# JorisAR/GDPathTracing

Measured on AMD Instinct MI355X. Metric: Mrays/sec at 1920x1080, 8 spp, 4 bounces, higher is better.
Workload: dtype f32

## Files before the change

gdpathtracing_amd/csrc/jpt_kernels_wf2.hip:

```cpp
#include <algorithm>
#include <cstdlib>

#include "jpt_trace_core.h"
#include "jpt_tie_walk.h"
#include "jpt_tuning.h"

#ifndef JPT_PRIMARY_WAVES
#define JPT_PRIMARY_WAVES 7
#endif

namespace jpt {

namespace {

constexpr int kBlock = kTraceBlock;
constexpr uint32_t kSegments = 256u * JPT_WAVES_PER_SIMD;
struct WfTune {
    int refill_idle;
    int primary_refill_idle;
    int node_min_lanes;
    int leaf_min_lanes;
    int inst_min_lanes;
    int phase_frac16;
    int tail_rounds;
    int tail_lanes;
};

template <bool COUNT, bool W4>
__device__ __forceinline__ bool walk_round(Traversal<COUNT, W4>& tr, bool active, const WideSceneDev& sc,
                                           const typename Traversal<COUNT, W4>::Stack& st, DevCounters& cnt, const WfTune& tune, uint32_t& steps)
{
    const int kNodeMinLanes = tune.node_min_lanes;
    const bool lane0 = (threadIdx.x & 63) == 0;
    if (COUNT && lane0) cnt.phase[0]++;
    const int na = __popcll(__ballot(active));
    const int cap = (na * tune.phase_frac16) >> 4;
    const int lmin = tune.leaf_min_lanes < cap ? tune.leaf_min_lanes : cap;
    const int imin = tune.inst_min_lanes < cap ? tune.inst_min_lanes : cap;
    for (int it = 0; it < 64; it++) {
        if (active && !tr.have && tr.sp > 0) tr.pop_next(st);
        const bool want = active && tr.wants_node();
        const unsigned long long m = __ballot(want);
        if (m == 0 || (it > 0 && __popcll(m) < kNodeMinLanes)) break;
        if (COUNT && lane0) {
            cnt.phase[1]++;
            cnt.phase[2] += (unsigned long long)__popcll(m);
        }
        if (want) tr.node_step(sc, st, cnt);
        if (COUNT && want) steps++;
    }
    bool wl = active && tr.wants_leaf();
    bool wi = active && tr.wants_instance();
    if (W4 && (tune.leaf_min_lanes > 1 || tune.inst_min_lanes > 1)) {
        const int nl = __popcll(__ballot(wl)), ni = __popcll(__ballot(wi));
        const bool nodes_left = __any(active && tr.wants_node()) || __any(active && !tr.have && tr.sp > 0);
        const bool run_l = nl >= lmin || !(nodes_left || ni >= imin);
        const bool run_i = ni >= imin || !(nodes_left || (run_l && nl > 0));
        wl = wl && run_l;
        wi = wi && run_i;
    }
    if (COUNT) {
        const int nl = __popcll(__ballot(wl)), ni = __popcll(__ballot(wi));
        if (lane0 && nl) {
            cnt.phase[3]++;
            cnt.phase[4] += (unsigned long long)nl;
        }
        if (lane0 && ni) {
            cnt.phase[5]++;
            cnt.phase[6] += (unsigned long long)ni;
        }
    }
    if (wl) tr.leaf_step(sc, cnt);
    if (wi) tr.instance_step(sc, st, cnt);
    if (COUNT && (wl || wi)) steps++;
    return active && tr.finished();
}

__device__ __forceinline__ bool in_mask(const unsigned long long m) { return __builtin_amdgcn_inverse_ballot_w64(m); }

template <bool COUNT, bool W4>
__device__ __forceinline__ unsigned long long walk_round_masked(Traversal<COUNT, W4>& tr, const unsigned long long act, const WideSceneDev& sc,
                                                                const typename Traversal<COUNT, W4>::Stack& st, DevCounters& cnt, const WfTune& tune,
                                                                uint32_t& steps)
{
    const int kNodeMinLanes = tune.node_min_lanes;
    const bool lane0 = (threadIdx.x & 63) == 0;
    const bool active = in_mask(act);
    if (COUNT && lane0) cnt.phase[0]++;
    const int na = __popcll(act);
    const int cap = (na * tune.phase_frac16) >> 4;
    const int lmin = tune.leaf_min_lanes < cap ? tune.leaf_min_lanes : cap;
    const int imin = tune.inst_min_lanes < cap ? tune.inst_min_lanes : cap;
    for (int it = 0; it < 64; it++) {
        if (active && !tr.have && tr.sp > 0) tr.template pop_next<true>(st);
        const bool want = active && tr.wants_node();
        const unsigned long long m = __ballot(want);
        if (m == 0 || (it > 0 && __popcll(m) < kNodeMinLanes)) break;
        if (COUNT && lane0) {
            cnt.phase[1]++;
            cnt.phase[2] += (unsigned long long)__popcll(m);
        }
        if (want) tr.node_step(sc, st, cnt);
        if (COUNT && want) steps++;
    }
    const unsigned long long hm = __ballot(tr.have), bm = __ballot(tr.in_blas);
    const unsigned long long lf = __ballot(tr.cur < 0), sm = __ballot(tr.sp > 0);
    const unsigned long long hv = act & hm;
    unsigned long long wlm = hv & lf & bm, wim = hv & lf & ~bm;
    if (W4 && (tune.leaf_min_lanes > 1 || tune.inst_min_lanes > 1)) {
        const int nl = __popcll(wlm), ni = __popcll(wim);
        const bool nodes_left = ((hv & ~lf) | (act & ~hm & sm)) != 0ull;
        const bool run_l = nl >= lmin || !(nodes_left || ni >= imin);
        const bool run_i = ni >= imin || !(nodes_left || (run_l && nl > 0));
        wlm = run_l ? wlm : 0ull;
        wim = run_i ? wim : 0ull;
    }
    if (COUNT) {
        const int nl = __popcll(wlm), ni = __popcll(wim);
        if (lane0 && nl) {
            cnt.phase[3]++;
            cnt.phase[4] += (unsigned long long)nl;
        }
        if (lane0 && ni) {
            cnt.phase[5]++;
            cnt.phase[6] += (unsigned long long)ni;
        }
    }
    const bool wl = in_mask(wlm), wi = in_mask(wim);
    if (wl) tr.leaf_step(sc, cnt);
    if (wi) tr.instance_step(sc, st, cnt);
    if (COUNT && (wl || wi)) steps++;
    return act & ~((hm & ~wlm) | wim) & ~sm;
}

typedef float jpt_v4f __attribute__((ext_vector_type(4)));
typedef uint32_t jpt_v4u __attribute__((ext_vector_type(4)));
__device__ __forceinline__ float4 stream_ld4(const float4* p)
{
    const jpt_v4f v = __builtin_nontemporal_load(reinterpret_cast<const jpt_v4f*>(p));
    return make_float4(v.x, v.y, v.z, v.w);
}
__device__ __forceinline__ void stream_st4(float4* p, const float4 v)
{
    jpt_v4f w;
    w.x = v.x; w.y = v.y; w.z = v.z; w.w = v.w;
    __builtin_nontemporal_store(w, reinterpret_cast<jpt_v4f*>(p));
}
__device__ __forceinline__ uint4 stream_ldu4(const uint4* p)
{
    const jpt_v4u v = __builtin_nontemporal_load(reinterpret_cast<const jpt_v4u*>(p));
    return make_uint4(v.x, v.y, v.z, v.w);
}
__device__ __forceinline__ void stream_stf(float* p, const float v) { __builtin_nontemporal_store(v, p); }
__device__ __forceinline__ uint32_t stream_ldu(const uint32_t* p) { return __builtin_nontemporal_load(p); }
__device__ __forceinline__ void stream_stu(uint32_t* p, const uint32_t v) { __builtin_nontemporal_store(v, p); }

constexpr uint32_t kHasRadiance = 0x80000000u;
constexpr uint32_t kPathMask = 0x7fffffffu;

struct Wf2Buffers {
    float4* ray_o[2];
    float4* ray_d[2];
    float4* hit_a;
    uint32_t* hit_b;
    float4* thr_q[2];
    float4* thr;
    float4* rad;
    uint32_t* fin8;
    float* first_depth;
    uint32_t* qcount;
    uint32_t* redo_count;
    float4* redo_rec;
    uint32_t redo_cap;
};

struct FastDiv {
    uint32_t d, m;
};
inline FastDiv make_fastdiv(uint32_t d) { return FastDiv{d ? d : 1u, d > 1u ? (uint32_t)(0x100000000ull / d) : 0xffffffffu}; }
__device__ __forceinline__ uint32_t fdiv(uint32_t n, const FastDiv& f)
{
    uint32_t q = __umulhi(n, f.m);
    const uint32_t r = n - q * f.d;
    return r >= f.d ? q + 1u : q;
}

struct Wf2Dims {
    int32_t tile_x0, tile_y0;
    int32_t tiles_x, tiles_y;
    int32_t full_tiles_x, full_tiles_y;
    uint32_t tiles_per_frame;
    uint32_t slots_per_frame;
    uint32_t n_chunks;
    uint32_t seg_cap;
    uint32_t run_shift;
    FastDiv by_tiles_x, by_full_tiles_x;
    FastDiv by_frames;
    int32_t acc_groups = 1;
};

__device__ __forceinline__ void slot_to_pixel(uint32_t slot, const Wf2Dims& dm, int& px, int& ly)
{
    const uint32_t tile = slot >> 6, lane = slot & 63u;
    const uint32_t ty = fdiv(tile, dm.by_tiles_x), tx = tile - ty * (uint32_t)dm.tiles_x;
    const uint32_t ix = lane & 7u, iy = lane >> 3;
    px = (int)((tx + (uint32_t)dm.tile_x0) * 8u + ix);
    ly = (int)((ty + (uint32_t)dm.tile_y0) * 8u + iy);
}

__device__ __forceinline__ void path_slot_frame(uint32_t path, const Wf2Dims& dm, uint32_t n_frames, uint32_t& slot, uint32_t& f)
{
    slot = fdiv(path, dm.by_frames);
    f = path - slot * n_frames;
}

// ... 99 lines not shown
                const uint32_t lim = want < room ? want : room;
                if (give && r < lim) {
                    tr.sp--;
                    pw(2u * (n_pool + r)) = top;
                    pw(2u * (n_pool + r) + 1u) = (int32_t)((tr.in_blas ? 1u : 0u) | (tr.cur_inst << 1));
                }
                const uint32_t given = (uint32_t)__popcll(gm);
                n_pool += given < lim ? given : lim;
            }
        }
        __builtin_amdgcn_fence(__ATOMIC_RELEASE, "wavefront");
        __builtin_amdgcn_wave_barrier();
    }
    if (COUNT) {
        for (int off = 32; off > 0; off >>= 1) my_steps += (uint32_t)__shfl_xor((int)my_steps, off);
        if (lane == 0) count_walk(cnt, my_steps);
    }
    const float best = wave_min_f(tr.hit.t);
    const unsigned long long win = __ballot(tr.hit.tri != kNone && tr.hit.t == best);
    TraceHit out;
    out.t = 1e9f;
    out.u = out.v = 0.0f;
    out.tri = out.inst = 0u;
    out.front = false;
    if (win && best < 1e9f) {
        unsigned long long pick = win;
        if (__popcll(win) > 1) {
            const bool mine = ((win >> lane) & 1ull) != 0ull;
            uint32_t kt = mine ? tr.hit.tri : 0u;
            for (int off = 32; off > 0; off >>= 1) {
                const uint32_t o = (uint32_t)__shfl_xor((int)kt, off);
                kt = o > kt ? o : kt;
            }
            const bool top = mine && tr.hit.tri == kt;
            uint32_t ki = top ? ((tr.hit.inst >> kInstBits) & kInstMask) : 0u;
            for (int off = 32; off > 0; off >>= 1) {
                const uint32_t o = (uint32_t)__shfl_xor((int)ki, off);
                ki = o > ki ? o : ki;
            }
            pick = __ballot(top && ((tr.hit.inst >> kInstBits) & kInstMask) == ki);
        }
        const int w = __ffsll((long long)pick) - 1;
        out.t = best;
        out.u = __shfl(tr.hit.u, w);
        out.v = __shfl(tr.hit.v, w);
        out.tri = (uint32_t)__shfl((int)tr.hit.tri, w);
        out.front = __shfl((int)tr.hit.front, w) != 0;
        const uint32_t wi = (uint32_t)__shfl((int)tr.hit.inst, w);
        const uint32_t found_in = (wi >> kInstBits) & kInstMask;
        const bool tied = __popcll(win) > 1 || (wi & kHitTied) != 0u;
        out.inst = found_in | (found_in << kInstBits) | (tied ? kHitTied : 0u);
    }
    return out;
}

template <bool COUNT>
__device__ __attribute__((noinline)) void coop_walk_call(const WideSceneDev* __restrict__ scp, int32_t* lds_col, int32_t* pool, float ox, float oy,
                                                         float oz, float dx, float dy, float dz, DevCounters* cntp, TraceHit* out)
{
    int32_t spill[kStackSpill + 2];
    const typename Traversal<COUNT, true>::Stack st{lds_col, spill, kTraceBlock, kStackLds - 2, kStackSpill + 2};
    const WideSceneDev sc = *scp;
    DevCounters none = {};
    *out = coop_walk<COUNT>(sc, st, pool, mk3(ox, oy, oz), mk3(dx, dy, dz), COUNT ? *cntp : none, (uint32_t)kTraceBlock);
}


#ifndef JPT_MAX_CHAIN
#define JPT_MAX_CHAIN 4
#endif
constexpr int kMaxChain = JPT_MAX_CHAIN;
template <bool COUNT, bool W4, bool TAIL>
__device__ __forceinline__ void trace_queue(const WideSceneDev& sc, const Wf2Buffers& wb, const Wf2Dims& dm, const int bounce, const WfTune& tune,
                                            const uint32_t seg0, const uint32_t (&end)[kMaxChain], const uint32_t n, int32_t* __restrict__ stack,
                                            uint32_t* __restrict__ s_cursor, DevCounters& cnt)
{
    const int lane = threadIdx.x & 63;
    int32_t spill[kStackSpill];
    const typename Traversal<COUNT, W4>::Stack my_stack{&stack[threadIdx.x], spill, kTraceBlock, kStackLds};
    uint32_t dry_rounds = 0;
    const float4* __restrict__ qo = wb.ray_o[bounce & 1];
    const float4* __restrict__ qd = wb.ray_d[bounce & 1];
    Traversal<COUNT, W4> tr;
    tr.have = tr.in_blas = false;
    tr.cur = 0;
    tr.sp = 0;
    unsigned long long act = 0ull, unsaved = 0ull;
    bool exhausted = false;
    size_t my_loc = 0;
    uint32_t walk_steps = 0;
    auto save_hit = [&]() {
        stream_st4(&wb.hit_a[my_loc], make_float4(tr.hit.t, tr.hit.u, tr.hit.v, __uint_as_float(tr.hit.tri)));
        stream_stu(&wb.hit_b[my_loc], tr.hit.inst | (tr.hit.front ? 0x80000000u : 0u));
    };

    for (;;) {
        const unsigned long long idle = ~act;
        const int n_idle = __popcll(idle);
        if (!exhausted && n_idle >= tune.refill_idle) {
            if (in_mask(unsaved)) save_hit();
            unsaved = 0ull;
            uint32_t start = 0;
            if (lane == 0) start = atomicAdd(s_cursor, (uint32_t)n_idle);
            start = (uint32_t)__builtin_amdgcn_readfirstlane((int)start);
            if (start + (uint32_t)n_idle >= n) exhausted = true;
            if (start < n) {
                const uint32_t idx = start + lanes_below(idle, lane);
                const unsigned long long fill = idle & __ballot(idx < n);
                if (in_mask(fill)) {
                    uint32_t k = 0, first = 0;
                    for (int j = 0; j < kMaxChain - 1; j++)
                        if (idx >= end[j]) {
                            k = (uint32_t)j + 1u;
                            first = end[j];
                        }
                    const size_t loc = (size_t)(seg0 + k) * dm.seg_cap + (idx - first);
                    const float4 ro = stream_ld4(&qo[loc]), rd = stream_ld4(&qd[loc]);
                    tr.begin(sc, mk3(ro.x, ro.y, ro.z), mk3(rd.x, rd.y, rd.z));
                    my_loc = loc;
                    walk_steps = 0;
                }
                act |= fill;
            }
        }
        if (act == 0ull) {
            if (exhausted) break;
            continue;
        }
        {
            const unsigned long long done = walk_round_masked<COUNT, W4>(tr, act, sc, my_stack, cnt, tune, walk_steps);
            act &= ~done;
            unsaved |= done;
            if (COUNT) {
                if (in_mask(done)) count_walk(cnt, walk_steps);
            }
            if constexpr (TAIL && W4) {
                if (exhausted && ++dry_rounds >= (uint32_t)tune.tail_rounds && __popcll(act) <= tune.tail_lanes) break;
            }
        }
    }
    if constexpr (TAIL && W4) {
        unsigned long long left = act;
        if (left) {
            if (in_mask(unsaved)) save_hit();
            unsaved = 0ull;
            const int wave_col = (int)(threadIdx.x & ~63u);
            while (left) {
                const int src = __ffsll((long long)left) - 1;
                left &= left - 1ull;
                TraceHit h;
                const WideSceneDev sc_tail = sc;
                coop_walk_call<COUNT>(&sc_tail, &stack[threadIdx.x], &stack[(kStackLds - 2) * kTraceBlock + wave_col], __shfl(tr.wo.x, src),
                                      __shfl(tr.wo.y, src), __shfl(tr.wo.z, src), __shfl(tr.wd.x, src), __shfl(tr.wd.y, src), __shfl(tr.wd.z, src),
                                      COUNT ? &cnt : nullptr, &h);
                if (lane == src) {
                    tr.hit = h;
                    save_hit();
                }
            }
        }
    }
    if (in_mask(unsaved)) save_hit();
}

template <bool COUNT, bool W4, bool TAIL = false>
__global__ __launch_bounds__(kBlock, JPT_WAVES_PER_SIMD) void wf2_trace(WideSceneDev sc, Wf2Buffers wb, Wf2Dims dm, int bounce, WfTune tune,
                                                    int chain, DevCounters* __restrict__ counters)
{
    __shared__ int32_t stack[kStackLds * kBlock];
    __shared__ uint32_t s_cursor;
    const uint32_t seg0 = blockIdx.x * (uint32_t)chain;
    uint32_t end[kMaxChain];
    uint32_t n = 0;
    for (int k = 0; k < kMaxChain; k++) {
        if (k < chain && seg0 + (uint32_t)k < kSegments) n += wb.qcount[(size_t)bounce * kSegments + seg0 + (uint32_t)k];
        end[k] = n;
    }
    if (n == 0) return;
    if (threadIdx.x == 0) s_cursor = 0;
    __syncthreads();
    DevCounters cnt = {};
    trace_queue<COUNT, W4, TAIL>(sc, wb, dm, bounce, tune, seg0, end, n, stack, &s_cursor, cnt);
    if (COUNT) flush_counters(cnt, counters);
}

constexpr float kCellMargin = 0.01f;
__device__ __forceinline__ bool sky_cells_at(const RefCamera& cam, float two_over_w, float two_over_h, float fx, float fy, float w_ref, float& w_out,
                                             float v[3], f3& d)
{
    d = raster_direction_approx(cam, two_over_w, two_over_h, fx, fy, w_out);
    const f3 c = mk3(0.0f, 0.0f, 0.0f) + mk3(1.0f, 1.0f, 1.0f) * sample_sky(d);
    v[0] = clamp_(c.x, 0.0f, 1.0f) * 255.0f + 0.5f;
    v[1] = clamp_(c.y, 0.0f, 1.0f) * 255.0f + 0.5f;
    v[2] = clamp_(c.z, 0.0f, 1.0f) * 255.0f + 0.5f;
    return (w_out * w_ref > 0.0f) && (d.y == d.y);
}
__device__ __forceinline__ float sky_interior_excess(const f3 c[4])
{
    float chord2 = 0.0f, ay = 0.0f;
    for (int i = 0; i < 4; i++) {
        ay = fmax_(ay, __builtin_fabsf(c[i].y));
        for (int j = i + 1; j < 4; j++) {
            const f3 e = c[i] - c[j];
            chord2 = fmax_(chord2, e.x * e.x + e.y * e.y + e.z * e.z);
        }
    }
    if (!(chord2 < 0.2f)) return 1e30f;
    const float theta2 = 1.1f * chord2;
    const float m = fmin_(1.0f, ay + __builtin_sqrtf(theta2));
    return 6.4f * 0.25f * theta2 * m;
}

__global__ __launch_bounds__(kBlock) void wf2_sky_tiles(Wf2Dims dm, FrameParams fp, RefCamera cam, uint32_t* __restrict__ tile_cell)
// ... 523 lines not shown
```

gdpathtracing_amd/csrc/jpt_trace_core.h:

```cpp
#pragma once

#include "jpt_kernels.h"
#include "jpt_shade.h"

namespace jpt {

constexpr int kTraceBlock = 256;
#ifndef JPT_STACK_LDS
#define JPT_STACK_LDS 20
#endif
#ifndef JPT_WAVES_PER_SIMD
#define JPT_WAVES_PER_SIMD 7
#endif
constexpr int kStackLds = JPT_STACK_LDS;
constexpr int kStackSpill = 76;
constexpr int32_t kSentinel = 0x7fffffff;

struct WideSceneDev {
    const WideNode* __restrict__ blas_nodes;
    const WideNode* __restrict__ tlas_nodes;
    const WideNodeQ* __restrict__ nodesq;
    const WideTri* __restrict__ tris;
    const WideInstance* __restrict__ instances;
    int32_t tlas_root;
    uint32_t n_instances;
    const ReachTri* __restrict__ reach_tri;
    const ReachInst* __restrict__ reach_inst;
};

__device__ __forceinline__ float4 ld4(const void* p) { return *reinterpret_cast<const float4*>(p); }

__device__ __forceinline__ float slab(const f3& o, const f3& rD, float mnx, float mny, float mnz, float mxx, float mxy, float mxz)
{
    const float tx1 = (mnx - o.x) * rD.x, tx2 = (mxx - o.x) * rD.x;
    float tmin = fmin_(tx1, tx2), tmax = fmax_(tx1, tx2);
    const float ty1 = (mny - o.y) * rD.y, ty2 = (mxy - o.y) * rD.y;
    tmin = fmax_(tmin, fmin_(ty1, ty2)), tmax = fmin_(tmax, fmax_(ty1, ty2));
    const float tz1 = (mnz - o.z) * rD.z, tz2 = (mxz - o.z) * rD.z;
    tmin = fmax_(tmin, fmin_(tz1, tz2)), tmax = fmin_(tmax, fmax_(tz1, tz2));
    return (tmax >= tmin && tmax > 0.0f) ? tmin : 1e30f;
}

constexpr int kInstBits = 15;
constexpr uint32_t kInstMask = (1u << kInstBits) - 1u;
constexpr uint32_t kHitTied = 1u << 30;

struct TraceHit {
    float t, u, v;
    uint32_t tri, inst;
    bool front;
};

template <bool COUNT, bool W4 = false, bool REACH = false>
struct Traversal {
    static constexpr bool kLean = W4;
    f3 wo, wd, wrD;
    f3 o, d, rD;
    f3 ood;
    f3 xrD;
    TraceHit hit;
    int32_t cur;
    int sp;
    uint32_t cur_inst;
    bool in_blas, have;

    struct Stack {
        int32_t* __restrict__ lds;
        int32_t* __restrict__ spill;
        int stride = kTraceBlock;
        int lds_entries = kStackLds;
        int spill_entries = kStackSpill;
    };

    __device__ __forceinline__ void push(const Stack& st, int32_t v)
    {
        if (sp < st.lds_entries) st.lds[sp * st.stride] = v;
        else if (sp < st.lds_entries + st.spill_entries) st.spill[sp - st.lds_entries] = v;
        sp++;
    }
    __device__ __forceinline__ int32_t pop(const Stack& st)
    {
        sp--;
        if (st.lds_entries <= 0) return sp < st.spill_entries ? st.spill[sp] : kSentinel;
        const int row = sp < st.lds_entries ? sp : st.lds_entries - 1;
        int32_t v = st.lds[row * st.stride];
        if (__builtin_expect(sp >= st.lds_entries, 0)) v = sp < st.lds_entries + st.spill_entries ? st.spill[sp - st.lds_entries] : kSentinel;
        return v;
    }

    __device__ __forceinline__ void begin(const WideSceneDev& sc, f3 ro, f3 rd)
    {
        wo = ro;
        wd = rd;
        o = ro;
        d = rd;
        set_level();
        wrD = (kLean && REACH) ? xrD : rD;
        hit.t = 1e9f;
        hit.u = hit.v = 0.0f;
        hit.tri = hit.inst = 0;
        hit.front = false;
        sp = 0;
        in_blas = false;
        cur_inst = 0;
        cur = sc.tlas_root;
        have = sc.n_instances != 0;
    }

    __device__ __forceinline__ void set_level()
    {
        if (kLean) {
            rD = mk3(__builtin_amdgcn_fmed3f(__builtin_amdgcn_rcpf(d.x), -kRcpClamp, kRcpClamp), __builtin_amdgcn_fmed3f(__builtin_amdgcn_rcpf(d.y), -kRcpClamp, kRcpClamp),
                     __builtin_amdgcn_fmed3f(__builtin_amdgcn_rcpf(d.z), -kRcpClamp, kRcpClamp));
            ood = mk3(-(o.x * rD.x), -(o.y * rD.y), -(o.z * rD.z));
            if (REACH) xrD = rcp3(d);
        } else {
            rD = rcp3(d);
        }
    }


    __device__ __forceinline__ bool wants_node() const { return have && cur >= 0; }
    __device__ __forceinline__ bool wants_leaf() const { return have && cur < 0 && in_blas; }
    __device__ __forceinline__ bool wants_instance() const { return have && cur < 0 && !in_blas; }
    __device__ __forceinline__ bool finished() const { return !have && sp == 0; }

    __device__ __forceinline__ void node_step4(const WideSceneDev& sc, const Stack& st, DevCounters& cnt)
    {
        const char* __restrict__ base = reinterpret_cast<const char*>(sc.nodesq);
        const uint32_t rec = (uint32_t)cur << 6;
        const float4 h0 = ld4(base + rec);
        const float4 h1 = ld4(base + (rec + 16u));
        const float4 h2 = ld4(base + (rec + 32u));
        const float4 cf = ld4(base + (rec + 48u));
        node_step4_rec(h0, h1, h2, cf, st, cnt);
    }
    __device__ __forceinline__ void node_step4_rec(const float4 h0, const float4 h1, const float4 h2, const float4 cf, const Stack& st, DevCounters& cnt)
    {
        if (COUNT) {
            if (in_blas) cnt.blas_expand++;
            else cnt.tlas_expand++;
        }
        const float ax = h0.w * rD.x, ay = h1.x * rD.y, az = h1.y * rD.z;
        const float bx = __builtin_fmaf(h0.x, rD.x, ood.x), by = __builtin_fmaf(h0.y, rD.y, ood.y), bz = __builtin_fmaf(h0.z, rD.z, ood.z);
        const float mx = __builtin_fmaf(kWalkSlackOverEps, __builtin_fabsf(ax), __builtin_fabsf(bx)) + __builtin_fabsf(ood.x);
        const float my = __builtin_fmaf(kWalkSlackOverEps, __builtin_fabsf(ay), __builtin_fabsf(by)) + __builtin_fabsf(ood.y);
        const float mz = __builtin_fmaf(kWalkSlackOverEps, __builtin_fabsf(az), __builtin_fabsf(bz)) + __builtin_fabsf(ood.z);
        const float nbx = __builtin_fmaf(-kWalkEps, mx, bx), fbx = __builtin_fmaf(kWalkEps, mx, bx);
        const float nby = __builtin_fmaf(-kWalkEps, my, by), fby = __builtin_fmaf(kWalkEps, my, by);
        const float nbz = __builtin_fmaf(-kWalkEps, mz, bz), fbz = __builtin_fmaf(kWalkEps, mz, bz);
        const bool negx = __float_as_int(d.x) < 0, negy = __float_as_int(d.y) < 0, negz = __float_as_int(d.z) < 0;
        const uint32_t lox = __float_as_uint(h1.z), loy = __float_as_uint(h1.w), loz = __float_as_uint(h2.x);
        const uint32_t hix = __float_as_uint(h2.y), hiy = __float_as_uint(h2.z), hiz = __float_as_uint(h2.w);
        const uint32_t nwx = negx ? hix : lox, fwx = negx ? lox : hix;
        const uint32_t nwy = negy ? hiy : loy, fwy = negy ? loy : hiy;
        const uint32_t nwz = negz ? hiz : loz, fwz = negz ? loz : hiz;
        int32_t r0 = __float_as_int(cf.x), r1 = __float_as_int(cf.y), r2 = __float_as_int(cf.z), r3 = __float_as_int(cf.w);
        constexpr uint32_t kInvalid = 0x7f800000u;
        const float tcur = hit.t;
        auto key = [&](int k, int32_t ch) -> uint32_t {
            const float qnx = (float)((nwx >> (8 * k)) & 255u), qny = (float)((nwy >> (8 * k)) & 255u), qnz = (float)((nwz >> (8 * k)) & 255u);
            const float qfx = (float)((fwx >> (8 * k)) & 255u), qfy = (float)((fwy >> (8 * k)) & 255u), qfz = (float)((fwz >> (8 * k)) & 255u);
            const float t_in = fmax_(fmax_(fmax_(__builtin_fmaf(qnx, ax, nbx), __builtin_fmaf(qny, ay, nby)), __builtin_fmaf(qnz, az, nbz)), 0.0f);
            const float t_out = fmin_(fmin_(fmin_(__builtin_fmaf(qfx, ax, fbx), __builtin_fmaf(qfy, ay, fby)), __builtin_fmaf(qfz, az, fbz)), tcur);
            return ((t_in <= t_out) & (ch != kEmptyChild)) ? __float_as_uint(t_in) : kInvalid;
        };
        uint32_t k0 = key(0, r0), k1 = key(1, r1), k2 = key(2, r2), k3 = key(3, r3);
        auto cswap = [](uint32_t& ka, uint32_t& kb, int32_t& ra, int32_t& rb) {
            const bool lt = ka < kb;
            const uint32_t klo = lt ? ka : kb, khi = lt ? kb : ka;
            const int32_t rlo = lt ? ra : rb, rhi = lt ? rb : ra;
            ka = klo; kb = khi; ra = rlo; rb = rhi;
        };
        cswap(k0, k1, r0, r1);
        cswap(k2, k3, r2, r3);
        cswap(k0, k2, r0, r2);
        cswap(k1, k3, r1, r3);
        cswap(k1, k2, r1, r2);
        have = k0 < kInvalid;
        cur = have ? r0 : cur;
        if (k1 < kInvalid) {
            if (k2 < kInvalid) {
                if (k3 < kInvalid) push(st, r3);
                push(st, r2);
            }
            push(st, r1);
        }
    }

    __device__ __forceinline__ void node_step(const WideSceneDev& sc, const Stack& st, DevCounters& cnt)
    {
        if (W4) {
            node_step4(sc, st, cnt);
            return;
        }
        const WideNode* n = (in_blas ? sc.blas_nodes : sc.tlas_nodes) + cur;
        const float4 a = ld4(&n->lmin[0]);
        const float4 b = ld4(&n->lmax[1]);
        const float4 c = ld4(&n->rmin[2]);
        const float4 e = ld4(&n->left);
        if (COUNT) {
            if (in_blas) cnt.blas_expand++;
            else cnt.tlas_expand++;
        }
        const float d1 = slab(o, rD, a.x, a.y, a.z, a.w, b.x, b.y);
        const float d2 = slab(o, rD, b.z, b.w, c.x, c.y, c.z, c.w);
        const int32_t left = __float_as_int(e.x), right = __float_as_int(e.y);
        const bool lv = d1 < hit.t, rv = d2 < hit.t;
        const bool left_first = d1 < d2;
        const int32_t near_ref = left_first ? left : right, far_ref = left_first ? right : left;
        const bool near_v = left_first ? lv : rv, far_v = left_first ? rv : lv;
        have = false;
        if (near_v) {
            if (far_v) push(st, far_ref);
            cur = near_ref;
            have = true;
        } else if (far_v) {
            cur = far_ref;
            have = true;
        }
    }

    __device__ __forceinline__ void leaf_step(const WideSceneDev& sc, DevCounters& cnt)
    {
        const uint32_t bits = (uint32_t)~cur;
        const uint32_t first = bits & kLeafFirstMask;
        const uint32_t count = (bits >> kLeafCountShift) + 1u;
        have = false;
        for (uint32_t i = 0; i < count; i++) {
            const uint32_t ti = first + i;
            const WideTri* tp = sc.tris + ti;
            const float4 q0 = ld4(&tp->v0[0]);
            const float4 q1 = ld4(&tp->e1[0]);
            const float4 q2 = ld4(&tp->e2[0]);
            if (COUNT) cnt.tri_tests++;
            const f3 v0 = mk3(q0.x, q0.y, q0.z), edge1 = mk3(q1.x, q1.y, q1.z), edge2 = mk3(q2.x, q2.y, q2.z);
            if (W4) {
                const f3 pvec = cross3(d, edge2);
                const float det = dot3(edge1, pvec);
                const float invDet = 1.0f / det;
                const f3 tvec = o - v0;
                const float u = dot3(tvec, pvec) * invDet;
                const f3 qvec = cross3(tvec, edge1);
                const float v = dot3(d, qvec) * invDet;
                const float t = dot3(edge2, qvec) * invDet;
                bool out = (__builtin_fabsf(det) < 1e-5f) | (u < 0.0f) | (u > 1.0f) | (v < 0.0f) | (u + v > 1.0f) |
                           (t < 0.0f) | (t > hit.t);
                if (REACH) {
                    if (!out && !reaches_triangle(sc, ti)) out = true;
                }
                float facing = dot3(mk3(q0.w, q1.w, q2.w), d);
                asm volatile("" : "+v"(facing));
                const bool front = facing > 0.0f;
                if (!out) {
                    const bool closer = t < hit.t;
                    hit.inst = ((closer ? cur_inst : hit.inst) & kInstMask) | (cur_inst << kInstBits) | (closer ? 0u : kHitTied);
                    hit.t = t;
                    hit.u = u;
                    hit.v = v;
                    hit.tri = ti;
                    hit.front = front;
                }
            } else {
                const f3 pvec = cross3(d, edge2);
                const float det = dot3(edge1, pvec);
                if (__builtin_fabsf(det) < 1e-5f) continue;
                const float invDet = 1.0f / det;
                const f3 tvec = o - v0;
                const float u = dot3(tvec, pvec) * invDet;
                if (u < 0.0f || u > 1.0f) continue;
                const f3 qvec = cross3(tvec, edge1);
                const float v = dot3(d, qvec) * invDet;
                if (v < 0.0f || u + v > 1.0f) continue;
                const float t = dot3(edge2, qvec) * invDet;
                if (t < 0.0f || t > hit.t) continue;
                if (REACH) {
                    if (!reaches_triangle(sc, ti)) continue;
                }
                hit.inst = (((t < hit.t) ? cur_inst : hit.inst) & kInstMask) | (cur_inst << kInstBits);
                hit.t = t;
                hit.u = u;
                hit.v = v;
                hit.tri = ti;
                hit.front = dot3(cross3(edge1, edge2), d) > 0.0f;
            }
        }
    }

    __device__ __forceinline__ bool reaches_triangle(const WideSceneDev& sc, uint32_t ti) const
    {
        const float4 a = ld4(&sc.reach_tri[ti].lo[0]), b = ld4(&sc.reach_tri[ti].hi[0]);
        if (__float_as_uint(a.w) != 0u) return true;
        return slab(o, kLean ? xrD : rD, a.x, a.y, a.z, b.x, b.y, b.z) < 1e30f;
    }

    __device__ __forceinline__ void instance_step(const WideSceneDev& sc, const Stack& st, DevCounters& cnt)
    {
        cur_inst = (uint32_t)~cur;
        if (REACH) {
            if (sc.n_instances > 1u) {
                const float4 a = ld4(&sc.reach_inst[cur_inst].lo[0]), b = ld4(&sc.reach_inst[cur_inst].hi[0]);
                if (!(slab(wo, wrD, a.x, a.y, a.z, b.x, b.y, b.z) < 1e30f)) {
                    if (kLean) {
                        o = wo;
                        d = wd;
                        set_level();
                    }
                    have = false;
                    return;
                }
            }
        }
        const WideInstance* ip = sc.instances + cur_inst;
        const float4 m0 = ld4(&ip->inv[0]);
        const float4 m1 = ld4(&ip->inv[4]);
        const float4 m2 = ld4(&ip->inv[8]);
        const int32_t root = ip->root;
        if (COUNT) cnt.inst_visits++;
        o = mk3(m0.x * wo.x + m0.w * wo.y + m1.z * wo.z + m2.y, m0.y * wo.x + m1.x * wo.y + m1.w * wo.z + m2.z,
                m0.z * wo.x + m1.y * wo.y + m2.x * wo.z + m2.w);
        d = mk3(m0.x * wd.x + m0.w * wd.y + m1.z * wd.z, m0.y * wd.x + m1.x * wd.y + m1.w * wd.z,
                m0.z * wd.x + m1.y * wd.y + m2.x * wd.z);
        set_level();
        in_blas = true;
        push(st, kSentinel);
        cur = root;
        have = true;
    }

    template <bool ON_DEMAND = false>
    __device__ __forceinline__ void pop_next(const Stack& st)
    {
        cur = pop(st);
        if (cur == kSentinel) {
            in_blas = false;
            if (sp == 0) return;
            cur = pop(st);
            if (!kLean || cur >= 0) {
                o = wo;
                d = wd;
                if (kLean && ON_DEMAND) asm volatile("" : "+v"(d.x), "+v"(d.y), "+v"(d.z));
                if (kLean) set_level();
                else rD = wrD;
            }
        }
        have = true;
    }

    __device__ __forceinline__ bool step(const WideSceneDev& sc, const Stack& st, DevCounters& cnt)
    {
        if (!have) {
            if (sp == 0) return false;
            pop_next(st);
            if (!have) return false;
        }
        if (cur >= 0) node_step(sc, st, cnt);
        else if (in_blas) leaf_step(sc, cnt);
        else instance_step(sc, st, cnt);
        return true;
    }
};

}
```

gdpathtracing_amd/csrc/jpt_wf2_paths.h:

```cpp
#if JPT_ENV >= 3
#if JPT_ENV == 4
#define JPT_ENV_NAME(name) name##_tx
#define JPT_LTOTAL (lt.n != 0u ? lt.marg[lt.n_blocks] : 0.0f)
#define JPT_MISS_WEIGHT env_miss_weight_tx
#define JPT_HIT_WEIGHT light_hit_weight_tx
#else
#define JPT_ENV_NAME(name) name##_lt
#define JPT_LTOTAL lt.marg[lt.n_blocks]
#define JPT_MISS_WEIGHT env_miss_weight
#define JPT_HIT_WEIGHT light_hit_weight
#endif
#define JPT_ENV_PARAM , EnvDev env, EnvSampDev es, LightDev lt, Wf2Nee nee, Wf2Nee lnee, int env_mode
#define JPT_ENV_ARG , env, es, lt, nee, lnee, env_mode
#define JPT_NEE_PARAM , bool& shadow, float4& so, float4& sd, float4& sc4, bool& lshadow, float4& lso, float4& lsd, float4& lsc
#define JPT_NEE_ARG , shadow, so, sd, sc4, lshadow, lso, lsd, lsc
#define JPT_SKY(d) (env_mode != 0 ? env_radiance(env, d) : sample_sky(d))
#define JPT_PDF lnee.pdf
#elif JPT_ENV == 2
#define JPT_ENV_NAME(name) name##_mis
#define JPT_ENV_PARAM , EnvDev env, EnvSampDev es, Wf2Nee nee
#define JPT_ENV_ARG , env, es, nee
#define JPT_NEE_PARAM , bool& shadow, float4& so, float4& sd, float4& sc4
#define JPT_NEE_ARG , shadow, so, sd, sc4
#define JPT_SKY(d) env_radiance(env, d)
#define JPT_PDF nee.pdf
#elif JPT_ENV
#define JPT_ENV_NAME(name) name##_env
#define JPT_ENV_PARAM , EnvDev env
#define JPT_ENV_ARG , env
#define JPT_NEE_PARAM
#define JPT_NEE_ARG
#define JPT_SKY(d) env_radiance(env, d)
#else
#define JPT_ENV_NAME(name) name
#define JPT_ENV_PARAM
#define JPT_ENV_ARG
#define JPT_NEE_PARAM
#define JPT_NEE_ARG
#define JPT_SKY(d) sample_sky(d)
#endif

#if JPT_ENV < 2


#ifdef JPT_LENS
#if JPT_ENV
#define JPT_PRIMARY_NAME wf2_primary_env_lens
#else
#define JPT_PRIMARY_NAME wf2_primary_lens
#endif
#define JPT_PRIMARY_PARAM LensDev lens
#elif defined(JPT_CAMERA_MODEL)
#if JPT_ENV
#define JPT_PRIMARY_NAME wf2_primary_env_cam
#else
#define JPT_PRIMARY_NAME wf2_primary_cam
#endif
#define JPT_PRIMARY_PARAM CamModelDev cm
#elif defined(JPT_BAKE)
#if JPT_ENV
#define JPT_PRIMARY_NAME wf2_primary_env_bake
#else
#define JPT_PRIMARY_NAME wf2_primary_bake
#endif
#define JPT_PRIMARY_PARAM BakeDev bake
#elif defined(JPT_PROBE)
#if JPT_ENV
#define JPT_PRIMARY_NAME wf2_primary_env_probe
#else
#define JPT_PRIMARY_NAME wf2_primary_probe
#endif
#define JPT_PRIMARY_PARAM ProbeDev probe
#elif defined(JPT_CUBE)
#if JPT_ENV
#define JPT_PRIMARY_NAME wf2_primary_env_cube
#else
#define JPT_PRIMARY_NAME wf2_primary_cube
#endif
#define JPT_PRIMARY_PARAM CubeDev cube
#else
#define JPT_PRIMARY_NAME JPT_ENV_NAME(wf2_primary)
#define JPT_PRIMARY_PARAM SkyCull cull
#endif

template <bool COUNT, bool W4, bool TAIL = false>
__global__ __launch_bounds__(kBlock, JPT_PRIMARY_WAVES) void JPT_PRIMARY_NAME(WideSceneDev sc, Wf2Buffers wb, Wf2Dims dm, FrameParams fp, RefCamera cam,
                                                      WfTune tune, JPT_PRIMARY_PARAM, DevCounters* __restrict__ counters)
{
    __shared__ int32_t stack[kStackLds * kBlock];
    __shared__ uint32_t s_cursor, s_out;
    const int lane = threadIdx.x & 63;
    const uint32_t seg = blockIdx.x;
    const uint32_t run_mask = (1u << dm.run_shift) - 1u;
    const uint32_t n_runs = (dm.n_chunks + run_mask) >> dm.run_shift;
    const uint32_t my_runs = seg < n_runs ? (n_runs - seg + kSegments - 1u) / kSegments : 0u;
    const uint32_t n = (my_runs << dm.run_shift) * 64u;
    if (threadIdx.x == 0) {
        s_cursor = 0;
        s_out = 0;
    }
    if ((int)threadIdx.x >= 1 && (int)threadIdx.x <= fp.max_bounces + 1) wb.qcount[(size_t)threadIdx.x * kSegments + seg] = 0u;
    if (seg == 0 && threadIdx.x >= 192u) wb.redo_count[threadIdx.x - 192u] = 0u;
    __syncthreads();
    int32_t spill[kStackSpill];
    const typename Traversal<COUNT, W4>::Stack my_stack{&stack[threadIdx.x], spill, kTraceBlock, kStackLds};
    const size_t seg_base = (size_t)seg * dm.seg_cap;
    uint32_t dry_rounds = 0;
    DevCounters cnt = {};
    Traversal<COUNT, W4> tr;
    bool active = false, exhausted = false;
    bool unsaved = false;
    uint32_t path = 0;
    uint32_t walk_steps = 0;
    auto save_results = [&]() {
#if JPT_ENV
        const bool is_hit = unsaved;
#else
        const bool is_hit = unsaved && tr.hit.t < 1e9f;
#endif
        const unsigned long long hm = __ballot(is_hit);
        if (hm) {
            uint32_t base = 0;
            if (lane == 0) base = atomicAdd(&s_out, (uint32_t)__popcll(hm));
            base = (uint32_t)__builtin_amdgcn_readfirstlane((int)base);
            if (is_hit) {
                const uint32_t j = base + lanes_below(hm, lane);
                stream_st4(&wb.ray_o[0][seg_base + j], make_float4(tr.wo.x, tr.wo.y, tr.wo.z, 0.0f));
                stream_st4(&wb.ray_d[0][seg_base + j], make_float4(tr.wd.x, tr.wd.y, tr.wd.z, __uint_as_float(path)));
                stream_st4(&wb.hit_a[seg_base + j], make_float4(tr.hit.t, tr.hit.u, tr.hit.v, __uint_as_float(tr.hit.tri)));
                stream_stu(&wb.hit_b[seg_base + j], tr.hit.inst | (tr.hit.front ? 0x80000000u : 0u));
            }
        }
#if !JPT_ENV
        if (unsaved && !is_hit) {
            uint32_t pslot, f;
            path_slot_frame(path, dm, (uint32_t)fp.n_frames, pslot, f);
            const f3 sky = mk3(0.0f, 0.0f, 0.0f) + mk3(1.0f, 1.0f, 1.0f) * JPT_SKY(tr.wd);
            store_final(wb, fp.accum_mode, path, sky);
            if ((int)f == fp.depth_frame) wb.first_depth[pslot] = cam.far_;
        }
#endif
        unsaved = false;
    };

    for (;;) {
        const unsigned long long idle = __ballot(!active);
        const int n_idle = __popcll(idle);
        if (!exhausted && n_idle >= tune.primary_refill_idle) {
            if (__any(unsaved)) save_results();
            uint32_t start = 0;
            if (lane == 0) start = atomicAdd(&s_cursor, (uint32_t)n_idle);
            start = (uint32_t)__builtin_amdgcn_readfirstlane((int)start);
            if (start + (uint32_t)n_idle >= n) exhausted = true;
            if (start < n && !active) {
                const uint32_t idx = start + lanes_below(idle, lane);
                if (idx < n) {
                    const uint32_t j = idx >> 6;
                    const uint32_t chunk = ((seg + (j >> dm.run_shift) * kSegments) << dm.run_shift) + (j & run_mask);
                    uint32_t slot = 0, f = 0;
                    if (chunk < dm.n_chunks) path_slot_frame(chunk * 64u + (idx & 63u), dm, (uint32_t)fp.n_frames, slot, f);
                    int px, ly;
                    slot_to_pixel(slot, dm, px, ly);
                    if (chunk < dm.n_chunks && px < fp.width && ly < fp.local_rows) {
                        const int py = local_to_global_row(ly, fp);
                        path = slot * (uint32_t)fp.n_frames + f;
                        if (COUNT) cnt.rays++;
#ifdef JPT_LENS
                        {
                            uint32_t sx, sy;
                            Ray ray = primary_ray(cam, fp.width, fp.height, px, py, fp.frame_index + f, sx, sy);
                            lens_ray(lens, sx, sy, ray);
#elif defined(JPT_CAMERA_MODEL)
                        {
                            uint32_t sx, sy;
                            const Ray ray = camera_ray(cam, cm, fp.width, fp.height, px, py, fp.frame_index + f, sx, sy);
#elif defined(JPT_BAKE)
                        const size_t texel = (size_t)py * (size_t)fp.width + (size_t)px;
                        const float4 bake_n = bake.normal[texel];
                        if (!bake_texel_valid(bake_n)) {
                            if (COUNT) cnt.rays--;
                            store_final(wb, fp.accum_mode, path, mk3(0.0f, 0.0f, 0.0f));
                            if ((int)f == fp.depth_frame) wb.first_depth[slot] = cam.far_;
                        } else {
// ... 665 lines not shown
```

Baseline: 28570.

## Track traversal have/in_blas state as wave masks and use LDS-address stack pointer

Replaces the per-lane booleans `have` and `in_blas` and the integer stack index in the wavefront trace queue with wave-wide 64-bit masks held in scalar registers. It also stores the traversal stack top as a raw LDS byte address, so push and pop skip the index-to-address arithmetic. Node, instance and pop steps gain a MASKED variant that writes the child key and top through a small struct, and the round logic derives the pop, node, leaf and instance sets from ballots. The aim is to cut per-lane VGPR use and divergent bookkeeping in the hot traversal loop. The cost is more ballot and scalar mask work and extra code complexity in the sentinel handling.

```diff
diff --git a/gdpathtracing_amd/csrc/jpt_kernels_wf2.hip b/gdpathtracing_amd/csrc/jpt_kernels_wf2.hip
--- a/gdpathtracing_amd/csrc/jpt_kernels_wf2.hip
+++ b/gdpathtracing_amd/csrc/jpt_kernels_wf2.hip
@@ -78,38 +78,59 @@
 
 __device__ __forceinline__ bool in_mask(const unsigned long long m) { return __builtin_amdgcn_inverse_ballot_w64(m); }
 
+struct WalkMasks {
+    unsigned long long have = 0ull, in_blas = 0ull;
+};
 template <bool COUNT, bool W4>
-__device__ __forceinline__ unsigned long long walk_round_masked(Traversal<COUNT, W4>& tr, const unsigned long long act, const WideSceneDev& sc,
+__device__ __forceinline__ unsigned long long walk_round_masked(Traversal<COUNT, W4>& tr, typename Traversal<COUNT, W4>::Masked& ml, WalkMasks& wm,
+                                                                const unsigned long long act, const WideSceneDev& sc,
                                                                 const typename Traversal<COUNT, W4>::Stack& st, DevCounters& cnt, const WfTune& tune,
                                                                 uint32_t& steps)
 {
+    using Walk = Traversal<COUNT, W4>;
     const int kNodeMinLanes = tune.node_min_lanes;
     const bool lane0 = (threadIdx.x & 63) == 0;
-    const bool active = in_mask(act);
     if (COUNT && lane0) cnt.phase[0]++;
     const int na = __popcll(act);
     const int cap = (na * tune.phase_frac16) >> 4;
     const int lmin = tune.leaf_min_lanes < cap ? tune.leaf_min_lanes : cap;
     const int imin = tune.inst_min_lanes < cap ? tune.inst_min_lanes : cap;
+    const uint32_t base = Walk::lds_base(st);
+    unsigned long long have_m = wm.have, blas_m = wm.in_blas;
     for (int it = 0; it < 64; it++) {
-        if (active && !tr.have && tr.sp > 0) tr.template pop_next<true>(st);
-        const bool want = active && tr.wants_node();
-        const unsigned long long m = __ballot(want);
+        const unsigned long long pm = act & ~have_m & __ballot(ml.top > base);
+        if (pm) {
+            if (in_mask(pm)) tr.cur = tr.pop_at(st, ml.top);
+            const unsigned long long sent = pm & __ballot(tr.cur == kSentinel);
+            have_m |= pm & ~sent;
+            if (sent) {
+                blas_m &= ~sent;
+                const unsigned long long more = sent & __ballot(ml.top > base);
+                if (in_mask(more)) {
+                    tr.cur = tr.pop_at(st, ml.top);
+                    if (!Walk::kLean || tr.cur >= 0) tr.restore_world();
+                }
+                have_m |= more;
+            }
+        }
+        const unsigned long long m = act & have_m & __ballot(tr.cur >= 0);
         if (m == 0 || (it > 0 && __popcll(m) < kNodeMinLanes)) break;
         if (COUNT && lane0) {
             cnt.phase[1]++;
             cnt.phase[2] += (unsigned long long)__popcll(m);
         }
-        if (want) tr.node_step(sc, st, cnt);
+        const bool want = in_mask(m);
+        ml.in_blas = in_mask(blas_m);
+        if (want) tr.template node_step<true>(sc, st, cnt, &ml);
         if (COUNT && want) steps++;
-    }
-    const unsigned long long hm = __ballot(tr.have), bm = __ballot(tr.in_blas);
-    const unsigned long long lf = __ballot(tr.cur < 0), sm = __ballot(tr.sp > 0);
-    const unsigned long long hv = act & hm;
-    unsigned long long wlm = hv & lf & bm, wim = hv & lf & ~bm;
+        have_m = (have_m & ~m) | (m & __ballot(ml.k0 < Walk::kNoChild));
+    }
+    const unsigned long long lf = __ballot(tr.cur < 0), sm = __ballot(ml.top > base);
+    const unsigned long long hv = act & have_m;
+    unsigned long long wlm = hv & lf & blas_m, wim = hv & lf & ~blas_m;
     if (W4 && (tune.leaf_min_lanes > 1 || tune.inst_min_lanes > 1)) {
         const int nl = __popcll(wlm), ni = __popcll(wim);
-        const bool nodes_left = ((hv & ~lf) | (act & ~hm & sm)) != 0ull;
+        const bool nodes_left = ((hv & ~lf) | (act & ~have_m & sm)) != 0ull;
         const bool run_l = nl >= lmin || !(nodes_left || ni >= imin);
         const bool run_i = ni >= imin || !(nodes_left || (run_l && nl > 0));
         wlm = run_l ? wlm : 0ull;
@@ -128,9 +149,13 @@
     }
     const bool wl = in_mask(wlm), wi = in_mask(wim);
     if (wl) tr.leaf_step(sc, cnt);
-    if (wi) tr.instance_step(sc, st, cnt);
+    if (wi) tr.template instance_step<true>(sc, st, cnt, &ml);
     if (COUNT && (wl || wi)) steps++;
-    return act & ~((hm & ~wlm) | wim) & ~sm;
+    have_m = (have_m & ~wlm) | wim;
+    blas_m |= wim;
+    wm.have = have_m;
+    wm.in_blas = blas_m;
+    return act & ~have_m & ~sm;
 }
 
 typedef float jpt_v4f __attribute__((ext_vector_type(4)));
@@ -396,9 +421,12 @@
     const float4* __restrict__ qo = wb.ray_o[bounce & 1];
     const float4* __restrict__ qd = wb.ray_d[bounce & 1];
     Traversal<COUNT, W4> tr;
-    tr.have = tr.in_blas = false;
     tr.cur = 0;
-    tr.sp = 0;
+    WalkMasks wm;
+    typename Traversal<COUNT, W4>::Masked ml;
+    ml.top = Traversal<COUNT, W4>::lds_base(my_stack);
+    ml.k0 = 0u;
+    ml.in_blas = false;
     unsigned long long act = 0ull, unsaved = 0ull;
     bool exhausted = false;
     size_t my_loc = 0;
@@ -431,10 +459,13 @@
                     const size_t loc = (size_t)(seg0 + k) * dm.seg_cap + (idx - first);
                     const float4 ro = stream_ld4(&qo[loc]), rd = stream_ld4(&qd[loc]);
                     tr.begin(sc, mk3(ro.x, ro.y, ro.z), mk3(rd.x, rd.y, rd.z));
+                    ml.top = Traversal<COUNT, W4>::lds_base(my_stack);
                     my_loc = loc;
                     walk_steps = 0;
                 }
                 act |= fill;
+                wm.have = sc.n_instances != 0 ? (wm.have | fill) : (wm.have & ~fill);
+                wm.in_blas &= ~fill;
             }
         }
         if (act == 0ull) {
@@ -442,7 +473,7 @@
             continue;
         }
         {
-            const unsigned long long done = walk_round_masked<COUNT, W4>(tr, act, sc, my_stack, cnt, tune, walk_steps);
+            const unsigned long long done = walk_round_masked<COUNT, W4>(tr, ml, wm, act, sc, my_stack, cnt, tune, walk_steps);
             act &= ~done;
             unsaved |= done;
             if (COUNT) {
diff --git a/gdpathtracing_amd/csrc/jpt_trace_core.h b/gdpathtracing_amd/csrc/jpt_trace_core.h
--- a/gdpathtracing_amd/csrc/jpt_trace_core.h
+++ b/gdpathtracing_amd/csrc/jpt_trace_core.h
@@ -86,6 +86,46 @@
         int32_t v = st.lds[row * st.stride];
         if (__builtin_expect(sp >= st.lds_entries, 0)) v = sp < st.lds_entries + st.spill_entries ? st.spill[sp - st.lds_entries] : kSentinel;
         return v;
+    }
+
+    typedef __attribute__((address_space(3))) int32_t LdsWord;
+    struct Masked {
+        uint32_t top;
+        uint32_t k0;
+        bool in_blas;
+    };
+    static constexpr uint32_t kNoChild = 0x7f800000u;
+    static __device__ __forceinline__ uint32_t lds_base(const Stack& st) { return (uint32_t)(uintptr_t)(LdsWord*)st.lds; }
+    static __device__ __forceinline__ uint32_t lds_limit(const Stack& st) { return lds_base(st) + (uint32_t)(st.lds_entries * st.stride) * 4u; }
+    static __device__ __forceinline__ LdsWord* lds_at(uint32_t a) { return (LdsWord*)(uintptr_t)a; }
+    __device__ __forceinline__ void push_at(const Stack& st, uint32_t& top, int32_t v) const
+    {
+        const uint32_t lim = lds_limit(st);
+        if (__builtin_expect(top < lim, 1)) *lds_at(top) = v;
+        else {
+            const int k = (int)((top - lim) / ((uint32_t)st.stride * 4u));
+            if (k < st.spill_entries) st.spill[k] = v;
+        }
+        top += (uint32_t)st.stride * 4u;
+    }
+    __device__ __forceinline__ int32_t pop_at(const Stack& st, uint32_t& top) const
+    {
+        const uint32_t lim = lds_limit(st), last = lim - (uint32_t)st.stride * 4u;
+        top -= (uint32_t)st.stride * 4u;
+        int32_t v = *lds_at(top < last ? top : last);
+        if (__builtin_expect(top >= lim, 0)) {
+            const int k = (int)((top - lim) / ((uint32_t)st.stride * 4u));
+            v = k < st.spill_entries ? st.spill[k] : kSentinel;
+        }
+        return v;
+    }
+    __device__ __forceinline__ void restore_world()
+    {
+        o = wo;
+        d = wd;
+        if (kLean) asm volatile("" : "+v"(d.x), "+v"(d.y), "+v"(d.z));
+        if (kLean) set_level();
+        else rD = wrD;
     }
 
     __device__ __forceinline__ void begin(const WideSceneDev& sc, f3 ro, f3 rd)
@@ -125,7 +165,8 @@
     __device__ __forceinline__ bool wants_instance() const { return have && cur < 0 && !in_blas; }
     __device__ __forceinline__ bool finished() const { return !have && sp == 0; }
 
-    __device__ __forceinline__ void node_step4(const WideSceneDev& sc, const Stack& st, DevCounters& cnt)
+    template <bool MASKED = false>
+    __device__ __forceinline__ void node_step4(const WideSceneDev& sc, const Stack& st, DevCounters& cnt, Masked* ms = nullptr)
     {
         const char* __restrict__ base = reinterpret_cast<const char*>(sc.nodesq);
         const uint32_t rec = (uint32_t)cur << 6;
@@ -133,12 +174,15 @@
         const float4 h1 = ld4(base + (rec + 16u));
         const float4 h2 = ld4(base + (rec + 32u));
         const float4 cf = ld4(base + (rec + 48u));
-        node_step4_rec(h0, h1, h2, cf, st, cnt);
-    }
-    __device__ __forceinline__ void node_step4_rec(const float4 h0, const float4 h1, const float4 h2, const float4 cf, const Stack& st, DevCounters& cnt)
-    {
+        node_step4_rec<MASKED>(h0, h1, h2, cf, st, cnt, ms);
+    }
+    template <bool MASKED = false>
+    __device__ __forceinline__ void node_step4_rec(const float4 h0, const float4 h1, const float4 h2, const float4 cf, const Stack& st, DevCounters& cnt,
+                                                   Masked* ms = nullptr)
+    {
+        static_assert(!(MASKED && REACH), "the masked rounds do not walk with reach records");
         if (COUNT) {
-            if (in_blas) cnt.blas_expand++;
+            if (MASKED ? ms->in_blas : in_blas) cnt.blas_expand++;
             else cnt.tlas_expand++;
         }
         const float ax = h0.w * rD.x, ay = h1.x * rD.y, az = h1.y * rD.z;
@@ -177,23 +221,37 @@
         cswap(k0, k2, r0, r2);
         cswap(k1, k3, r1, r3);
         cswap(k1, k2, r1, r2);
-        have = k0 < kInvalid;
-        cur = have ? r0 : cur;
-        if (k1 < kInvalid) {
-            if (k2 < kInvalid) {
-                if (k3 < kInvalid) push(st, r3);
-                push(st, r2);
-            }
-            push(st, r1);
-        }
-    }
-
-    __device__ __forceinline__ void node_step(const WideSceneDev& sc, const Stack& st, DevCounters& cnt)
+        if constexpr (MASKED) {
+            ms->k0 = k0;
+            cur = k0 < kInvalid ? r0 : cur;
+            if (k1 < kInvalid) {
+                if (k2 < kInvalid) {
+                    if (k3 < kInvalid) push_at(st, ms->top, r3);
+                    push_at(st, ms->top, r2);
+                }
+                push_at(st, ms->top, r1);
+            }
+        } else {
+            have = k0 < kInvalid;
+            cur = have ? r0 : cur;
+            if (k1 < kInvalid) {
+                if (k2 < kInvalid) {
+                    if (k3 < kInvalid) push(st, r3);
+                    push(st, r2);
+                }
+                push(st, r1);
+            }
+        }
+    }
+
+    template <bool MASKED = false>
+    __device__ __forceinline__ void node_step(const WideSceneDev& sc, const Stack& st, DevCounters& cnt, Masked* ms = nullptr)
     {
         if (W4) {
-            node_step4(sc, st, cnt);
+            node_step4<MASKED>(sc, st, cnt, ms);
             return;
         }
+        const bool in_blas = MASKED ? ms->in_blas : this->in_blas;
         const WideNode* n = (in_blas ? sc.blas_nodes : sc.tlas_nodes) + cur;
         const float4 a = ld4(&n->lmin[0]);
         const float4 b = ld4(&n->lmax[1]);
@@ -210,14 +268,24 @@
         const bool left_first = d1 < d2;
         const int32_t near_ref = left_first ? left : right, far_ref = left_first ? right : left;
         const bool near_v = left_first ? lv : rv, far_v = left_first ? rv : lv;
-        have = false;
-        if (near_v) {
-            if (far_v) push(st, far_ref);
-            cur = near_ref;
-            have = true;
-        } else if (far_v) {
-            cur = far_ref;
-            have = true;
+        if constexpr (MASKED) {
+            if (near_v) {
+                if (far_v) push_at(st, ms->top, far_ref);
+                cur = near_ref;
+            } else if (far_v) {
+                cur = far_ref;
+            }
+            ms->k0 = (near_v || far_v) ? 0u : kNoChild;
+        } else {
+            have = false;
+            if (near_v) {
+                if (far_v) push(st, far_ref);
+                cur = near_ref;
+                have = true;
+            } else if (far_v) {
+                cur = far_ref;
+                have = true;
+            }
         }
     }
 
@@ -294,8 +362,10 @@
         return slab(o, kLean ? xrD : rD, a.x, a.y, a.z, b.x, b.y, b.z) < 1e30f;
     }
 
-    __device__ __forceinline__ void instance_step(const WideSceneDev& sc, const Stack& st, DevCounters& cnt)
-    {
+    template <bool MASKED = false>
+    __device__ __forceinline__ void instance_step(const WideSceneDev& sc, const Stack& st, DevCounters& cnt, Masked* ms = nullptr)
+    {
+        static_assert(!(MASKED && REACH), "the masked rounds do not walk with reach records");
         cur_inst = (uint32_t)~cur;
         if (REACH) {
             if (sc.n_instances > 1u) {
@@ -322,10 +392,15 @@
         d = mk3(m0.x * wd.x + m0.w * wd.y + m1.z * wd.z, m0.y * wd.x + m1.x * wd.y + m1.w * wd.z,
                 m0.z * wd.x + m1.y * wd.y + m2.x * wd.z);
         set_level();
-        in_blas = true;
-        push(st, kSentinel);
-        cur = root;
-        have = true;
+        if constexpr (MASKED) {
+            push_at(st, ms->top, kSentinel);
+            cur = root;
+        } else {
+            in_blas = true;
+            push(st, kSentinel);
+            cur = root;
+            have = true;
+        }
     }
 
     template <bool ON_DEMAND = false>
diff --git a/gdpathtracing_amd/csrc/jpt_wf2_paths.h b/gdpathtracing_amd/csrc/jpt_wf2_paths.h
--- a/gdpathtracing_amd/csrc/jpt_wf2_paths.h
+++ b/gdpathtracing_amd/csrc/jpt_wf2_paths.h
@@ -99,6 +99,8 @@
         s_cursor = 0;
         s_out = 0;
     }
+    static_assert(kBlock >= 192 + 64, "threads 192 .. 255 of block 0 clear the 64 set-aside words");
+    static_assert(kMaxBounces + 1 < 192, "threads 1 .. max_bounces + 1 clear the queue-size rows: they must end below thread 192");
     if ((int)threadIdx.x >= 1 && (int)threadIdx.x <= fp.max_bounces + 1) wb.qcount[(size_t)threadIdx.x * kSegments + seg] = 0u;
     if (seg == 0 && threadIdx.x >= 192u) wb.redo_count[threadIdx.x - 192u] = 0u;
     __syncthreads();
```

Result: faster. 28950, median of 6 (+1.3%).
